# CederGroupHub/chgnet

Hardware: AMD Instinct MI355X
Metric: structures/s (energy+force+stress) on batched ~50-atom crystals (higher is better)
Workload: dtype f32; 1 GPU; 1024 x LiMnO2 5x1x1 (40 atoms, sigma=0.01 frac perturbation) per GPU, task efs; structures_per_gpu=1024, atoms=40960, directed_bonds=3535504, angles=4125764, bond_graph_nodes=213755, weights=random-init 0.3.0 architecture (tests/golden/weights_seed0.npz), parallelism=structures sharded over 1 GPU(s), RCCL all-gather of energies only, process_group_ranks=1, energies_in_all_gather=1024, comm=none (single rank)

## Files before the change

chgnet_amd/csrc/engine.hip:

```cpp

#include "engine_internal.h"
#include <cstring>

namespace chgh {

template <int UNROLL>
__global__ __launch_bounds__(256) void k_stream_copy(const f32x4* __restrict__ src, f32x4* __restrict__ dst, size_t n) {
  const size_t stride = (size_t)gridDim.x * blockDim.x;
  size_t i = (size_t)blockIdx.x * blockDim.x + threadIdx.x;
  for (; i + (UNROLL - 1) * stride < n; i += UNROLL * stride) {
    f32x4 v[UNROLL];
#pragma unroll
    for (int u = 0; u < UNROLL; ++u) v[u] = __builtin_nontemporal_load(src + i + u * stride);
#pragma unroll
    for (int u = 0; u < UNROLL; ++u) __builtin_nontemporal_store(v[u], dst + i + u * stride);
  }
  for (; i < n; i += stride) dst[i] = src[i];
}

template <bool NT>
__global__ __launch_bounds__(256) void k_stream_copy_seg(const f32x4* __restrict__ src, f32x4* __restrict__ dst, size_t n) {
  constexpr size_t SEG = 1024;
  const size_t nseg = n / SEG;
  for (size_t sgm = blockIdx.x; sgm < nseg; sgm += gridDim.x) {
// ... 78 lines not shown
  if (eng->desc.n_mlp_hidden == 0) eng->desc.n_mlp_hidden = 3;
  if (eng->desc.n_mlp_hidden != 2 && eng->desc.n_mlp_hidden != 3) {
    eng->err = "n_mlp_hidden = " + std::to_string(desc->n_mlp_hidden) + ": the energy head has two or three hidden layers";
    return CHG_EUNSUPPORTED;
  }
  if (const char* g = std::getenv("CHGNET_HIP_GRAPHS")) eng->use_graphs = std::string(g) != "0";
  if (const char* g = std::getenv("CHGNET_WIDE_RANGE")) eng->force_wide = std::string(g) == "1";
  if (const char* g = std::getenv("CHGNET_SPEC_BUILD")) eng->spec_builds = std::string(g) != "0";
  HIP_TRY(eng, hipSetDevice(device));
  hipDeviceProp_t prop;
  HIP_TRY(eng, hipGetDeviceProperties(&prop, device));
  if (std::string(prop.gcnArchName).rfind("gfx950", 0) != 0) {
    eng->err = std::string("device is ") + prop.gcnArchName + ", this library contains gfx950 code only";
    return CHG_ENODEV;
  }
  eng->num_cus = prop.multiProcessorCount;
  HIP_TRY(eng, hipStreamCreateWithFlags(&eng->stream, hipStreamNonBlocking));
  HIP_TRY(eng, hipStreamCreateWithFlags(&eng->copy_stream, hipStreamNonBlocking));
  HIP_TRY(eng, hipEventCreate(&eng->t0));
  HIP_TRY(eng, hipEventCreate(&eng->t1));
  Weights probe{};
  const size_t need = layout_weights(nullptr, desc->n_conv, probe);
  if ((int64_t)need != desc->n_weights) {
    eng->err = "weight blob has " + std::to_string(desc->n_weights) + " floats, layout needs " + std::to_string(need);
    return CHG_EINVAL;
  }
  HIP_TRY(eng, hipMalloc(&eng->d_weights, need * sizeof(float)));
  if (int rs = check_weight_range(eng, weights_blob, need); rs != CHG_OK) { eng->err = "chg_engine_create: " + eng->err; *out = eng; return rs; }
  HIP_TRY(eng, hipMemcpy(eng->d_weights, weights_blob, need * sizeof(float), hipMemcpyHostToDevice));
  layout_weights(eng->d_weights, desc->n_conv, eng->w);
  { const int si = build_images(eng); if (si) return si; }
  { int s; if ((s = predict_set_lds(eng)) || (s = chgh_wide::predict_set_lds(eng)) || (s = train_set_lds(eng)) || (s = chgh_wide::train_set_lds(eng))) return s; }
  return CHG_OK;
}

int chg_engine_destroy(chg_engine* eng) {
  if (!eng) return CHG_OK;
  hipSetDevice(eng->device);
  if (eng->stream) hipStreamSynchronize(eng->stream);
  for (auto& pe : eng->pending) { hipEventDestroy(pe.start); hipEventDestroy(pe.stop); }
  for (auto e : eng->event_pool) hipEventDestroy(e);
  if (eng->t0) hipEventDestroy(eng->t0);
  if (eng->t1) hipEventDestroy(eng->t1);
  for (auto& a : eng->arena_pool) hipFree(a.first);
  for (auto& a : eng->work_pool) hipFree(a.first);
  if (eng->scratch) hipFree(eng->scratch);
  if (eng->h_stage) hipHostFree(eng->h_stage);
  if (eng->h_out) hipHostFree(eng->h_out);
  if (eng->d_weights) hipFree(eng->d_weights);
  if (eng->d_images) hipFree(eng->d_images);
  if (eng->copy_stream) hipStreamDestroy(eng->copy_stream);
  if (eng->stream) hipStreamDestroy(eng->stream);
  delete eng;
  return CHG_OK;
}

const char* chg_last_error(const chg_engine* eng) { return eng ? eng->err.c_str() : "null engine"; }

int chg_engine_build_stats(chg_engine* eng, int64_t* single_pass_builds, int64_t* capacity_overflows) {
  if (!eng) return CHG_EINVAL;
  if (single_pass_builds) *single_pass_builds = eng->n_spec_builds;
  if (capacity_overflows) *capacity_overflows = eng->n_spec_overflows;
  return CHG_OK;
}

int chg_engine_set_graph_search(chg_engine* eng, int32_t search, int32_t cell_min_atoms) {
  if (!eng || search < 0 || search > 2 || cell_min_atoms < 0) return CHG_EINVAL;
  eng->graph_search = search;
  if (cell_min_atoms > 0) eng->cell_min_atoms = cell_min_atoms;
  return CHG_OK;
}

int chg_engine_cell_stats(chg_engine* eng, int64_t* cell_builds, int64_t* all_pairs_fallbacks) {
  if (!eng) return CHG_EINVAL;
  if (cell_builds) *cell_builds = eng->n_cell_builds;
  if (all_pairs_fallbacks) *all_pairs_fallbacks = eng->n_cell_fallbacks;
  return CHG_OK;
}

int chg_engine_set_memory_limit(chg_engine* eng, int64_t bytes) {
  if (!eng || bytes < 0) return CHG_EINVAL;
  eng->memory_limit = (size_t)bytes;
  return CHG_OK;
}

int chg_engine_memory_info(chg_engine* eng, int64_t* free_bytes, int64_t* total_bytes) {
  if (!eng) return CHG_EINVAL;
  HIP_TRY(eng, hipSetDevice(eng->device));
  size_t f = 0, t = 0;
  HIP_TRY(eng, hipMemGetInfo(&f, &t));
  std::lock_guard<std::mutex> lk(eng->pool_mu);
  for (auto& a : eng->arena_pool) f += a.second;
  for (auto& a : eng->work_pool) f += a.second;
  if (free_bytes) *free_bytes = (int64_t)f;
  if (total_bytes) *total_bytes = (int64_t)t;
  return CHG_OK;
}

int64_t chg_batch_bytes_required(int32_t n_conv, int32_t n_struct, int32_t n_atoms, int32_t n_directed, int32_t n_angles, int32_t n_bnodes) {
  if (n_conv < 2 || n_conv > MAX_CONV || n_struct < 0 || n_atoms < 0 || n_directed < 0 || (n_directed & 1) || n_angles < 0 || n_bnodes < 0) return -1;
  chg_batch probe{};
  probe.B = n_struct; probe.N = n_atoms; probe.Ed = n_directed; probe.Eu = n_directed / 2; probe.A = n_angles; probe.Eb = n_bnodes; probe.L = n_conv;
  probe.blk_cap = upload_blk_cap(probe.N, probe.A, probe.Eb);
  size_t total = 0;
  carve(&probe, nullptr, total);
  return (int64_t)total;
}

int chg_batch_upload(chg_engine* eng, const chg_batch_host* h, chg_batch** out) {
  if (!eng || !h || !out) return CHG_EINVAL;
  if (h->n_struct <= 0 || h->n_atoms <= 0 || h->n_directed < 0 || h->n_directed != 2 * h->n_undirected || h->n_angles < 0 ||
      h->n_bnodes < 0 || (h->n_angles > 0 && h->n_bnodes == 0)) {
    eng->err = "chg_batch_upload: inconsistent counts";
    return CHG_EINVAL;
  }
  HIP_TRY(eng, hipSetDevice(eng->device));
  chg_batch* b = new (std::nothrow) chg_batch();
  if (!b) return CHG_ENOMEM;
  b->B = h->n_struct; b->N = h->n_atoms; b->Ed = h->n_directed; b->Eu = h->n_undirected; b->A = h->n_angles; b->Eb = h->n_bnodes;
  b->L = eng->desc.n_conv;
  b->blk_cap = upload_blk_cap(b->N, b->A, b->Eb);
  size_t total = 0;
  carve(b, nullptr, total);
  {
    const int sa = acquire_arena(eng, b, total);
    if (sa != CHG_OK) { delete b; return sa; }
  }
  carve(b, b->arena, total);
  if (h->atom_off) b->h_atom_off.assign(h->atom_off, h->atom_off + h->n_struct + 1);
  b->h_volume.resize(h->n_struct);
  for (int q = 0; q < h->n_struct; ++q) {
    const float* Lf = h->lattice + 9 * q;
    b->h_volume[q] = Lf[0] * (Lf[4] * Lf[8] - Lf[5] * Lf[7]) + Lf[1] * (Lf[5] * Lf[6] - Lf[3] * Lf[8]) + Lf[2] * (Lf[3] * Lf[7] - Lf[4] * Lf[6]);
  }
  int s = CHG_OK;
  const size_t B = b->B, N = b->N, Ed = b->Ed, Eu = b->Eu, A = b->A, Eb = b->Eb;
#define UP(field, n) if (s == CHG_OK) s = h2d(eng, b->field, h->field, (n), eng->copy_stream)
  UP(z, N); UP(atom_owner, N); UP(atom_off, B + 1); UP(frac, 3 * N); UP(lattice, 9 * B);
  UP(e_center, Ed); UP(e_nbr, Ed); UP(e_d2u, Ed); UP(e_owner, Ed); UP(e_image, 3 * Ed); UP(e_rev, Ed); UP(p_center, Ed); UP(p_nbr, Ed);
  UP(u_u2d, Eu); UP(u_bnode, Eu); UP(bn_und, Eb);
  UP(a_ctr, A); UP(a_b1c, A); UP(a_b2c, A); UP(a_d1, A); UP(a_d2, A);
#undef UP
  b->win_pending = true;
  if (s == CHG_OK && hipStreamSynchronize(eng->copy_stream) != hipSuccess) { eng->err = "chg_batch_upload: sync failed"; s = CHG_EHIP; }
  if (s != CHG_OK) { hipFree(b->arena); delete b; return s; }
  *out = b;
  return CHG_OK;
}

int chg_debug_fetch_i32(chg_engine* eng, chg_batch* b, const char* name, int32_t* dst, int64_t capacity, int64_t* n_written) {
  if (!eng || !b || !name || !dst) return CHG_EINVAL;
  if (std::strcmp(name, "wide_range") == 0) {
    if (capacity >= 1) dst[0] = b->wide_range ? 1 : 0;
    if (n_written) *n_written = capacity >= 1 ? 1 : 0;
    return CHG_OK;
  }
  if (std::strcmp(name, "route") == 0) {
    const int64_t n = std::min<int64_t>(6, std::max<int64_t>(capacity, 0));
    std::copy(b->route, b->route + n, dst);
    if (n_written) *n_written = n;
    return CHG_OK;
  }
  if (b->named_i32.empty()) register_names(b);
  auto it = b->named_i32.find(name);
  if (it == b->named_i32.end()) { eng->err = std::string("chg_debug_fetch_i32: unknown buffer ") + name; return CHG_EINVAL; }
  const size_t n = std::min<size_t>(it->second.second, (size_t)std::max<int64_t>(capacity, 0));
  TRY(ensure_windows(eng, b));
  HIP_TRY(eng, hipStreamSynchronize(eng->stream));
  if (n) HIP_TRY(eng, hipMemcpy(dst, it->second.first, n * sizeof(int32_t), hipMemcpyDeviceToHost));
  if (n_written) *n_written = (int64_t)n;
  return CHG_OK;
}

int chg_batch_update_geometry(chg_engine* eng, chg_batch* b, const float* frac, const float* lattice) {
  if (!eng || !b) return CHG_EINVAL;
  HIP_TRY(eng, hipSetDevice(eng->device));
  int s = CHG_OK;
  if (frac) s = h2d(eng, b->frac, frac, (size_t)3 * b->N);
  if (s == CHG_OK && lattice) {
    s = h2d(eng, b->lattice, lattice, (size_t)9 * b->B);
    b->h_volume.resize(b->B);
    for (int q = 0; q < b->B; ++q) {
      const float* Lf = lattice + 9 * (size_t)q;
      b->h_volume[q] = Lf[0] * (Lf[4] * Lf[8] - Lf[5] * Lf[7]) + Lf[1] * (Lf[5] * Lf[6] - Lf[3] * Lf[8]) + Lf[2] * (Lf[3] * Lf[7] - Lf[4] * Lf[6]);
    }
  }
  b->q_tables = false;
  if (s == CHG_OK) HIP_TRY(eng, hipStreamSynchronize(eng->stream));
  return s;
}

int chg_batch_free(chg_engine* eng, chg_batch* b) {
  if (!b) return CHG_OK;
  if (eng) { hipSetDevice(eng->device); hipStreamSynchronize(eng->stream); }
  if (b->graph_exec) hipGraphExecDestroy(b->graph_exec);
  release_workspace(eng, b->train_arena, b->train_bytes, 0);
  release_workspace(eng, b->t2_arena, b->t2_bytes, 1);
  free_train2(b);
  if (b->arena) {
    bool pooled = false;
    if (eng) {
      std::lock_guard<std::mutex> lk(eng->pool_mu);
      if (eng->arena_pool.size() < 2) { eng->arena_pool.emplace_back(b->arena, b->arena_bytes); pooled = true; }
    }
    if (!pooled) hipFree(b->arena);
  }
  delete b;
  return CHG_OK;
}

int64_t chg_batch_device_bytes(const chg_batch* b) { return b ? (int64_t)b->arena_bytes : 0; }

int chg_predict(chg_engine* eng, chg_batch* b, uint32_t task_mask) {
  if (!eng || !b) return CHG_EINVAL;
  HIP_TRY(eng, hipSetDevice(eng->device));
  const uint32_t task = task_mask | CHG_TASK_E;
  TRY(ensure_windows(eng, b));
  if (eng->force_wide) b->wide_range = true;
  if (b->wide_range) return chgh_wide::run_predict(eng, b, task);
  if (eng->profiling || !eng->use_graphs) return run_predict(eng, b, task);
  if (b->graph_task != task) {
    if (b->graph_exec) hipGraphExecDestroy(b->graph_exec);
    b->graph_exec = nullptr;
    b->graph_task = task;
    b->eager_calls = 0;
  }
  if (!b->graph_exec && b->eager_calls++ == 0) return run_predict(eng, b, task);
  if (!b->graph_exec) {
    hipGraph_t graph = nullptr;
    HIP_TRY(eng, hipStreamBeginCapture(eng->stream, hipStreamCaptureModeThreadLocal));
    const int s = run_predict(eng, b, task);
    const hipError_t e = hipStreamEndCapture(eng->stream, &graph);
    if (s != CHG_OK) { if (graph) hipGraphDestroy(graph); return s; }
    if (e != hipSuccess) { eng->err = std::string("hipStreamEndCapture: ") + hipGetErrorString(e); return CHG_EHIP; }
    const hipError_t ei = hipGraphInstantiate(&b->graph_exec, graph, nullptr, nullptr, 0);
    hipGraphDestroy(graph);
    if (ei != hipSuccess) { b->graph_exec = nullptr; eng->err = std::string("hipGraphInstantiate: ") + hipGetErrorString(ei); return CHG_EHIP; }
    b->graph_task = task;
    std::copy(b->route, b->route + 6, b->graph_route);
  }
  HIP_TRY(eng, hipGraphLaunch(b->graph_exec, eng->stream));
  std::copy(b->graph_route, b->graph_route + 6, b->route);
  b->last_task = task;
  b->seed1_adjoints = (task & (CHG_TASK_F | CHG_TASK_S)) != 0;
  b->q_tables = b->seed1_adjoints;
  return CHG_OK;
}

int chg_engine_update_weights(chg_engine* eng, const float* weights_blob) {
  if (!eng || !weights_blob) return CHG_EINVAL;
  TRY(check_weight_range(eng, weights_blob, (size_t)eng->desc.n_weights));
  HIP_TRY(eng, hipSetDevice(eng->device));
  HIP_TRY(eng, hipMemcpyAsync(eng->d_weights, weights_blob, sizeof(float) * (size_t)eng->desc.n_weights, hipMemcpyHostToDevice, eng->stream));
  TRY(build_images(eng));
  HIP_TRY(eng, hipStreamSynchronize(eng->stream));
  return CHG_OK;
}

int chg_batch_all_gather_energy(chg_engine* eng, chg_batch* b, chg_comm* comm, int64_t width, float* table) {
  if (!eng || !b || !comm || !table || width < b->B) return CHG_EINVAL;
  if (b->last_task == 0) { eng->err = "chg_batch_all_gather_energy: run chg_predict on this batch first"; return CHG_EINVAL; }
  HIP_TRY(eng, hipSetDevice(eng->device));
  int32_t nranks = 1, comm_dev = -1;
  float* stage = nullptr;
  if (chg_comm_info(comm, nullptr, &nranks, &comm_dev) == CHG_OK && comm_dev != eng->device) {
    eng->err = "chg_batch_all_gather_energy: the communicator belongs to device " + std::to_string(comm_dev) + ", the engine to device " + std::to_string(eng->device);
    return CHG_EINVAL;
  }
  if (chg_comm_info(comm, nullptr, &nranks, nullptr) != CHG_OK || chg_comm_reserve(comm, width * (int64_t)(nranks + 1), &stage) != CHG_OK) {
    eng->err = std::string("chg_batch_all_gather_energy: ") + chg_comm_last_error(comm);
    return CHG_EHIP;
  }
  hipStream_t st = eng->stream;
  HIP_TRY(eng, hipMemsetAsync(stage, 0, sizeof(float) * (size_t)width, st));
  HIP_TRY(eng, hipMemcpyAsync(stage, b->energy, sizeof(float) * (size_t)b->B, hipMemcpyDeviceToDevice, st));
  if (chg_comm_all_gather_f32_device(comm, stage, width, stage + width, st) != CHG_OK) {
    eng->err = std::string("chg_batch_all_gather_energy: ") + chg_comm_last_error(comm);
    return CHG_EHIP;
  }
  HIP_TRY(eng, hipMemcpyAsync(table, stage + width, sizeof(float) * (size_t)width * nranks, hipMemcpyDeviceToHost, st));
  HIP_TRY(eng, hipStreamSynchronize(st));
  return CHG_OK;
}

void* chg_engine_stream(chg_engine* eng) { return eng ? static_cast<void*>(eng->stream) : nullptr; }
int chg_engine_device(chg_engine* eng) { return eng ? eng->device : -1; }

int chg_synchronize(chg_engine* eng) {
  if (!eng) return CHG_EINVAL;
  HIP_TRY(eng, hipStreamSynchronize(eng->stream));
  if (eng->profiling) return collect_profile(eng);
  return CHG_OK;
}

int chg_batch_download(chg_engine* eng, chg_batch* b, const chg_out_host* o) {
  if (!eng || !b || !o) return CHG_EINVAL;
  HIP_TRY(eng, hipSetDevice(eng->device));
  const size_t B = b->B, N = b->N;
  struct Piece { float* dst; const float* src; size_t n; };
  const Piece pieces[] = {
      {o->energy, b->energy, B},
      {(b->last_task & CHG_TASK_F) ? o->force : nullptr, b->force, 3 * N},
      {(b->last_task & CHG_TASK_S) ? o->stress : nullptr, b->virial, 9 * B},
      {(b->last_task & CHG_TASK_M) ? o->magmom : nullptr, b->magmom, N},
      {o->site_energy, b->site_energy, N},
      {o->atom_fea, b->atom[b->L - 1], N * D},
// ... 203 lines not shown
```

chgnet_amd/csrc/kernels_conv.h:

```cpp
#pragma once

#include "mfma_tile.h"
#include "mfma_split.h"

namespace chg {

constexpr int TS = 2 * D + PAD;
constexpr int WS = D + PAD;
constexpr int TILE_FLOATS = TILE_ROWS * TS;
constexpr int VEC_SLOTS = 6;
constexpr int IMG64 = 1024, IMG128 = 2048;
constexpr int angle_split(bool hidden, bool bwd) { return (hidden && bwd) ? 2 : 1; }

struct GatedW {
  const float *w2c, *b2c, *w2g, *b2g, *ln1_g, *ln1_b, *ln2_g, *ln2_b;
};

__device__ __forceinline__ void stage_gated_vecs(float* vecs, const GatedW& gw, bool hidden, int tid) {
  if (hidden) {
    stage_vector(vecs + 0 * D, gw.b2c, D, tid);
    stage_vector(vecs + 1 * D, gw.b2g, D, tid);
  }
  stage_vector(vecs + 2 * D, gw.ln1_g, D, tid);
  stage_vector(vecs + 3 * D, gw.ln1_b, D, tid);
// ... 354 lines not shown
    if (i >= g.n) return;
    if (y < g.p[i].col_blocks) {
      if (K == 128 && g.p[i].x2_off > 0) rows_gemm_body<K, NOUT, (K == 128 ? 2 : 1)>(g.p[i], y);
      else rows_gemm_body<K, NOUT, 1>(g.p[i], y);
      return;
    }
    y -= g.p[i].col_blocks;
  }
}

template <int K, int NOUT, int PARTS = 1>
constexpr size_t rows_gemm_lds() {
  return sizeof(float) * (PARTS * NOUT * (K + PAD) + NOUT + WAVES * TILE_ROWS * ((K > NOUT ? K : NOUT) + PAD));
}

struct AtomConvArgs {
  const float* P;
  const float* Q;
  const float* wag;
  const int *e_center, *e_nbr, *e_d2u;
  int n_edges;
  GatedW gw;
  const float *hb0, *hbc;
  const int* u_bnode;
  const float *w_bond, *q_bias;
  float* Qout;
  const float* image;
  float* agg;
  const float* GA;
  float* GP;
  float* GQ;
  float* Gwag;
  int first_wag;
  float* Gb;
  int gb_accumulate;
  float* dumpG;
  float* dumpH;
  float* g_ln;
};

constexpr int AC_VEC_SLOTS = VEC_SLOTS + 2;
template <int NW = WAVES, bool BWD = false, bool FUSEQ = false>
constexpr size_t atomconv_lds() {
  if (FUSEQ) return 16 * (size_t)(2 * IMG64 + IMG128) + sizeof(float) * (AC_VEC_SLOTS * D + NW * TILE_FLOATS);
  return 16 * (size_t)(BWD ? 4 : 2) * IMG64 + sizeof(float) * (VEC_SLOTS * D + NW * TILE_FLOATS);
}

constexpr int ac_fwd_image_floats() { return 4 * (2 * IMG64 + IMG128) + AC_VEC_SLOTS * D; }
__device__ __forceinline__ void atomconv_fwd_stage(float* base, const AtomConvArgs& p, int tid, int nthreads) {
  h16x8* I2c = reinterpret_cast<h16x8*>(base);
  h16x8* I2g = I2c + IMG64;
  h16x8* Ib = I2g + IMG64;
  float* vecs = reinterpret_cast<float*>(Ib + IMG128);
  stage_split<false>(I2c, p.gw.w2c, D, D, tid, nthreads);
  stage_split<false>(I2g, p.gw.w2g, D, D, tid, nthreads);
  stage_split<false>(Ib, p.w_bond, 2 * D, D, tid, nthreads);
  stage_gated_vecs(vecs, p.gw, true, tid);
  for (int q = tid; q < 2 * D; q += nthreads) vecs[VEC_SLOTS * D + q] = p.q_bias ? p.q_bias[q] : 0.f;
}
__device__ __forceinline__ void atomconv_bwd_stage(float* base, const AtomConvArgs& p, int tid, int nthreads) {
  h16x8* I2c = reinterpret_cast<h16x8*>(base);
  h16x8* I2g = I2c + IMG64;
  h16x8* I2cT = I2g + IMG64;
  h16x8* I2gT = I2cT + IMG64;
  float* vecs = reinterpret_cast<float*>(I2gT + IMG64);
  stage_split<false>(I2c, p.gw.w2c, D, D, tid, nthreads);
  stage_split<false>(I2g, p.gw.w2g, D, D, tid, nthreads);
  stage_split<true>(I2cT, p.gw.w2c, D, D, tid, nthreads);
  stage_split<true>(I2gT, p.gw.w2g, D, D, tid, nthreads);
  stage_gated_vecs(vecs, p.gw, true, tid);
}
constexpr int AC_RM_IMG = (int)(rm_image_bytes(D, D) / 4);
constexpr int ac_bwd_rm_image_floats() { return 2 * AC_RM_IMG + VEC_SLOTS * D + 4 * IMG128; }
__device__ __forceinline__ void atomconv_bwd_stage_rm(float* base, const AtomConvArgs& p, int tid, int nthreads) {
  stage_rm(reinterpret_cast<_Float16*>(base), p.gw.w2c, D, D, tid, nthreads);
  stage_rm(reinterpret_cast<_Float16*>(base + AC_RM_IMG), p.gw.w2g, D, D, tid, nthreads);
  float* vecs = base + 2 * AC_RM_IMG;
  stage_gated_vecs(vecs, p.gw, true, tid);
  stage_split<true>(reinterpret_cast<h16x8*>(vecs + VEC_SLOTS * D), p.w_bond, 2 * D, D, tid, nthreads);
}
template <int UNUSED = 0>
__global__ __launch_bounds__(BLOCK) void k_atomconv_image(AtomConvArgs p, float* out) { atomconv_fwd_stage(out, p, threadIdx.x, BLOCK); }
static __global__ __launch_bounds__(BLOCK) void k_atomconv_image_rm(AtomConvArgs p, float* out) { atomconv_bwd_stage_rm(out, p, threadIdx.x, BLOCK); }

__device__ __forceinline__ int bond_node(const AtomConvArgs& p, int k) { return p.hbc ? p.u_bnode[k] : -1; }
template <bool A32 = false>
__device__ __forceinline__ long bond_row_offset(const AtomConvArgs& p, int k, int bn) {
  if constexpr (A32) return (long)(bn >= 0 ? (unsigned)(p.hbc - p.hb0) + (unsigned)bn * D : (unsigned)k * D);
  else return bn >= 0 ? (p.hbc - p.hb0) + (long)bn * D : (long)k * D;
}

template <int NW, bool A32 = false>
__global__ __launch_bounds__(64 * NW) CHG_TWO_WAVES void k_atomconv_fwd(AtomConvArgs p) {
  extern __shared__ __attribute__((aligned(16))) float smem[];
  h16x8* I2c = reinterpret_cast<h16x8*>(smem);
  h16x8* I2g = I2c + IMG64;
  h16x8* Ib = I2g + IMG64;
  float* vecs = reinterpret_cast<float*>(Ib + IMG128);
  float* tiles = vecs + AC_VEC_SLOTS * D;
  const float* W2c = reinterpret_cast<const float*>(I2c);
  const float* W2g = reinterpret_cast<const float*>(I2g);
  const int tid = threadIdx.x, wave = tid >> 6, lane = tid & 63, j = lane & 15, g = lane >> 4;
  float* T = tiles + wave * TILE_FLOATS;
  float* Trow = T + j * TS;
  const int ntiles = (p.n_edges + TILE_ROWS - 1) / TILE_ROWS;
  const TileSeq ts = wave_tile_seq<true>(ntiles, NW, wave);
  const int tstride = TILE_ROWS;
  auto row_of = [&](int v) { return max(0, min(ts.at(v) * tstride + j, p.n_edges - 1)); };
  GatherPH gr;
  V64 wv_nx;
  int c_nx = 0, n_nx = 0, c_n2 = 0, n_n2 = 0;
  int bn_nx = -1, bn_n2 = -1;
  if (ts.count > 0) {
    const int r0 = row_of(0);
    c_nx = p.e_center[r0]; n_nx = p.e_nbr[r0];
    bn_nx = bond_node(p, r0 >> 1);
    gather_issue_ph<A32>(gr, p.P, c_nx, p.P + 2 * D, n_nx, 4 * D, 4 * D, p.hb0, bond_row_offset<A32>(p, r0 >> 1, bn_nx), lane);
    read_dl_g<VT, A32>(p.wag, (unsigned)(r0 >> 1), D, g, wv_nx.t);
    const int r1 = row_of(1);
    c_n2 = p.e_center[r1]; n_n2 = p.e_nbr[r1];
    bn_n2 = bond_node(p, r1 >> 1);
  }
  stage_image<ac_fwd_image_floats() / 4, 64 * NW>(smem, p.image, tid);
  __syncthreads();
  for (int v = 0; v < ts.count; ++v) {
    const int row0 = ts.at(v) * tstride;
    const int nvalid = min(TILE_ROWS, p.n_edges - row0);
    const int c = c_nx;
    const bool node = bn_nx >= 0;
    const V64 wv = wv_nx;
    gather_commit_h(gr, T, TS, lane);
    __builtin_amdgcn_wave_barrier();
    V64 x;
    read_dl<VT>(Trow, g, x.t);
    __builtin_amdgcn_wave_barrier();
    gather_commit_p(gr, T, TS, lane);
    __builtin_amdgcn_wave_barrier();
    c_nx = c_n2; n_nx = n_n2; bn_nx = bn_n2;
    if (v + 1 < ts.count) {
      const int r1 = row_of(v + 1);
      gather_issue_ph<A32>(gr, p.P, c_nx, p.P + 2 * D, n_nx, 4 * D, 4 * D, p.hb0, bond_row_offset<A32>(p, r1 >> 1, bn_nx), lane);
      read_dl_g<VT, A32>(p.wag, (unsigned)(r1 >> 1), D, g, wv_nx.t);
      const int r2 = row_of(v + 2);
      c_n2 = p.e_center[r2]; n_n2 = p.e_nbr[r2];
      bn_n2 = bond_node(p, r2 >> 1);
    }
    f32x4 z[2 * VT];
    if (!node) {
      read_dl<2 * VT>(vecs + VEC_SLOTS * D, g, z);
    } else {
#pragma unroll
      for (int ft = 0; ft < 2 * VT; ++ft) z[ft] = f32x4{0.f, 0.f, 0.f, 0.f};
    }
    gemm_split<VT, 2 * VT, false, true>(z, Ib, 2 * D, x.t, j, g);
    if (p.Qout && !(j & 1) && j < nvalid) {
      write_dl_g<2 * VT, A32>(p.Qout, (unsigned)((row0 + j) >> 1), 2 * D, g, z);
    }
    {
      f32x4 ps[2 * VT];
      read_dl<2 * VT>(Trow, g, ps);
#pragma unroll
      for (int ft = 0; ft < 2 * VT; ++ft) z[ft] += ps[ft];
    }
    V64 zc{{z[0], z[1], z[2], z[3]}}, zg{{z[4], z[5], z[6], z[7]}};
    GatedState s;
    V64 y;
    gated_forward<true, false, false, 1, true>(zc, zg, W2c, W2g, vecs, j, g, s, y);
    gather_take(gr);
    asm volatile("" : "+v"(c_n2), "+v"(n_n2), "+v"(bn_n2));
    CHG_EV(ft) asm volatile("" : "+v"(wv_nx.t[ft]));
    __builtin_amdgcn_wave_barrier();
    V64 m;
    CHG_EV(ft) m.t[ft] = y.t[ft] * wv.t[ft];
    write_dl<VT>(Trow, g, m.t);
    __builtin_amdgcn_wave_barrier();
    {
      float acc1 = 0.f, acc2 = 0.f;
      int cur1 = __builtin_amdgcn_readlane(c, 0), cur2 = __builtin_amdgcn_readlane(c, 1);
#pragma unroll
      for (int b = 0; b < TILE_ROWS / 2; ++b) {
        if (2 * b < nvalid) {
          const int c1 = __builtin_amdgcn_readlane(c, 2 * b), c2 = __builtin_amdgcn_readlane(c, 2 * b + 1);
          if (c1 != cur1) {
            tile_atomic_add(grow<float, A32>(p.agg, (unsigned)cur1, D, lane), acc1);
            acc1 = 0.f;
            cur1 = c1;
          }
          if (c2 != cur2) {
            tile_atomic_add(grow<float, A32>(p.agg, (unsigned)cur2, D, lane), acc2);
            acc2 = 0.f;
            cur2 = c2;
          }
          acc1 += T[(2 * b) * TS + lane];
          acc2 += T[(2 * b + 1) * TS + lane];
        }
      }
      tile_atomic_add(grow<float, A32>(p.agg, (unsigned)cur1, D, lane), acc1);
      tile_atomic_add(grow<float, A32>(p.agg, (unsigned)cur2, D, lane), acc2);
    }
    __builtin_amdgcn_wave_barrier();
  }
}

template <bool STORE_GQ = true, bool A32 = false>
__device__ __forceinline__ void acbwd_scatter(const float* T, int c, int nvalid, int k0, const AtomConvArgs& p, int lane) {
  float a1[4] = {0.f, 0.f, 0.f, 0.f}, a2[4] = {0.f, 0.f, 0.f, 0.f};
  int cur1 = __builtin_amdgcn_readlane(c, 0), cur2 = __builtin_amdgcn_readlane(c, 1);
#pragma unroll
  for (int b = 0; b < TILE_ROWS / 2; ++b) {
    if (2 * b < nvalid) {
      const float e0 = T[(2 * b) * TS + lane], e1 = T[(2 * b) * TS + 64 + lane];
      const float o0 = T[(2 * b + 1) * TS + lane], o1 = T[(2 * b + 1) * TS + 64 + lane];
      if (STORE_GQ) {
        float* q = p.GQ + (size_t)(k0 + b) * 2 * D + lane;
        q[0] = e0 + o0;
        q[64] = e1 + o1;
      }
      const int c1 = __builtin_amdgcn_readlane(c, 2 * b), c2 = __builtin_amdgcn_readlane(c, 2 * b + 1);
      if (c1 != cur1) {
        float* d = grow<float, A32>(p.GP, (unsigned)cur1, 4 * D, lane);
        tile_atomic_add(d, a1[0]); tile_atomic_add(d + 64, a1[1]); tile_atomic_add(d + 128, a1[2]); tile_atomic_add(d + 192, a1[3]);
        a1[0] = a1[1] = a1[2] = a1[3] = 0.f;
        cur1 = c1;
      }
      if (c2 != cur2) {
        float* d = grow<float, A32>(p.GP, (unsigned)cur2, 4 * D, lane);
        tile_atomic_add(d, a2[0]); tile_atomic_add(d + 64, a2[1]); tile_atomic_add(d + 128, a2[2]); tile_atomic_add(d + 192, a2[3]);
        a2[0] = a2[1] = a2[2] = a2[3] = 0.f;
        cur2 = c2;
      }
      a1[0] += e0; a1[1] += e1; a1[2] += o0; a1[3] += o1;
      a2[0] += o0; a2[1] += o1; a2[2] += e0; a2[3] += e1;
    }
  }
  float* d1 = grow<float, A32>(p.GP, (unsigned)cur1, 4 * D, lane);
  tile_atomic_add(d1, a1[0]); tile_atomic_add(d1 + 64, a1[1]); tile_atomic_add(d1 + 128, a1[2]); tile_atomic_add(d1 + 192, a1[3]);
  float* d2 = grow<float, A32>(p.GP, (unsigned)cur2, 4 * D, lane);
  tile_atomic_add(d2, a2[0]); tile_atomic_add(d2 + 64, a2[1]); tile_atomic_add(d2 + 128, a2[2]); tile_atomic_add(d2 + 192, a2[3]);
}

template <bool TRAIN, bool A32 = false>
__global__ __launch_bounds__(BLOCK) CHG_TWO_WAVES void k_atomconv_bwd(AtomConvArgs p) {
  constexpr bool FUSE_GQ = !TRAIN;
  constexpr int NW = WAVES;
  constexpr bool RM = FUSE_GQ;
  extern __shared__ __attribute__((aligned(16))) float smem[];
  constexpr int HMODE = RM ? 2 : 1;
  float* vecs = RM ? smem + 2 * AC_RM_IMG : smem + 4 * 4 * IMG64;
  const h16x8* IbT = reinterpret_cast<const h16x8*>(vecs + VEC_SLOTS * D);
  float* tiles = vecs + VEC_SLOTS * D + (FUSE_GQ ? 4 * IMG128 : 0);
  const float* W2c = smem;
  const float* W2g = RM ? smem + AC_RM_IMG : smem + 4 * IMG64;
  const float* W2cT = RM ? W2c : smem + 2 * 4 * IMG64;
  const float* W2gT = RM ? W2g : smem + 3 * 4 * IMG64;
  const int tid = threadIdx.x, lane = tid & 63, j = lane & 15, g = lane >> 4;
  const int wave = __builtin_amdgcn_readfirstlane(tid >> 6);
  float* T = tiles + wave * TILE_FLOATS;
  float* Trow = T + j * TS;
  const int ntiles = (p.n_edges + TILE_ROWS - 1) / TILE_ROWS;
  const TileSeq ts = wave_tile_seq<!TRAIN>(ntiles, NW, wave);
  const int last_row = p.n_edges - 1;
  int c, n, k;
  {
    const int row = max(0, min(ts.at(0) * TILE_ROWS + j, last_row));
    c = p.e_center[row]; n = p.e_nbr[row]; k = row >> 1;
    GatherRegs gr;
    gather_issue128<A32>(gr, p.P, c, p.P + 2 * D, n, p.Q, k, 4 * D, 4 * D, 2 * D, lane);
    if (TRAIN) atomconv_bwd_stage(smem, p, tid, 64 * NW);
    else stage_image<ac_bwd_rm_image_floats() / 4, 64 * NW>(smem, p.image, tid);
    gather_commit128(gr, T, TS, lane);
  }
  __syncthreads();
  TrainTile tt{};
  tt.T = T; tt.lane = lane;
  for (int v = 0; v < ts.count; ++v) {
    const int row0 = ts.at(v) * TILE_ROWS;
    const int nvalid = min(TILE_ROWS, p.n_edges - row0);
    if (TRAIN) {
      tt.nvalid = nvalid;
      tt.hrow = j < nvalid ? p.dumpH + (size_t)(row0 + j) * 2 * D : nullptr;
      tt.grow = j < nvalid ? p.dumpG + (size_t)(row0 + j) * 2 * D : nullptr;
    }
    int cn, nn, kn;
    {
      const int row = max(0, min(ts.at(v + 1) * TILE_ROWS + j, last_row));
      cn = p.e_center[row]; nn = p.e_nbr[row]; kn = row >> 1;
    }
    V64 wv, gm;
    read_dl_g<VT, A32>(p.wag, (unsigned)k, D, g, wv.t);
    read_dl_g<VT, A32>(p.GA, (unsigned)c, D, g, gm.t);
    const int k0 = row0 >> 1, nb = nvalid >> 1;
    float* gwag_rows = grow<float, A32>(p.Gwag, (unsigned)k0, D, lane);
    float prev[TILE_ROWS / 2];
#pragma unroll
    for (int b = 0; b < TILE_ROWS / 2; ++b) prev[b] = p.first_wag ? 0.f : gwag_rows[(size_t)min(b, nb - 1) * D];
    __builtin_amdgcn_wave_barrier();
    V64 zc, zg;
    read_dl<VT>(Trow, g, zc.t);
    read_dl<VT>(Trow + D, g, zg.t);
    GatedState s;
    V64 y;
    gated_forward<true, false, TRAIN, HMODE>(zc, zg, W2c, W2g, vecs, j, g, s, y, &tt);
    asm volatile("" : "+v"(cn), "+v"(nn));
    V64 gy, gw, gzc, gzg;
    CHG_EV(ft) {
      gw.t[ft] = gm.t[ft] * y.t[ft];
      gy.t[ft] = gm.t[ft] * wv.t[ft];
    }
    __builtin_amdgcn_wave_barrier();
    write_dl<VT>(Trow, g, gw.t);
    __builtin_amdgcn_wave_barrier();
    {
      float* dst = gwag_rows;
#pragma unroll
      for (int b = 0; b < TILE_ROWS / 2; ++b) prev[b] += T[(2 * b) * TS + lane] + T[(2 * b + 1) * TS + lane];
      if (nvalid == TILE_ROWS) {
#pragma unroll
        for (int b = 0; b < TILE_ROWS / 2; ++b) dst[(size_t)b * D] = prev[b];
      } else {
#pragma unroll
        for (int b = 0; b < TILE_ROWS / 2; ++b)
          if (b < nb) dst[(size_t)b * D] = prev[b];
      }
    }
    gated_backward<true, false, TRAIN, HMODE>(gy, zc, zg, W2cT, W2gT, vecs, j, g, s, gzc, gzg, &tt);
    if (FUSE_GQ) {
      float* gb_row = grow<float, A32>(p.Gb, (unsigned)(k0 + (j >> 1)), D, 4 * g);
      const bool owner = !(j & 1) && j < nvalid;
      V64 old = zero64();
      if (p.gb_accumulate && owner) {
        CHG_EV(ft) old.t[ft] = *reinterpret_cast<const f32x4*>(gb_row + 16 * ft);
      }
      f32x4 gz[2 * VT] = {gzc.t[0], gzc.t[1], gzc.t[2], gzc.t[3], gzg.t[0], gzg.t[1], gzg.t[2], gzg.t[3]};
      V64 gq = zero64();
      gemm_split<2 * VT, VT, true>(gq.t, IbT, D, gz, j, g);
      CHG_EW(ft, r) gq.t[ft][r] += __shfl_xor(gq.t[ft][r], 1);
      CHG_EV(ft) gq.t[ft] += old.t[ft];
      CHG_EV(ft) asm volatile("" : "+v"(gq.t[ft]));
      if (owner) {
        CHG_EV(ft) *reinterpret_cast<f32x4*>(gb_row + 16 * ft) = gq.t[ft];
      }
    }
    __builtin_amdgcn_wave_barrier();
    write_dl<VT>(Trow, g, gzc.t);
    write_dl<VT>(Trow + D, g, gzg.t);
    __builtin_amdgcn_wave_barrier();
    if (v + 1 < ts.count) {
      GatherRegs gr;
      gather_issue128<A32>(gr, p.P, cn, p.P + 2 * D, nn, p.Q, kn, 4 * D, 4 * D, 2 * D, lane);
      acbwd_scatter<!FUSE_GQ, A32>(T, c, nvalid, k0, p, lane);
      __builtin_amdgcn_wave_barrier();
      gather_commit128(gr, T, TS, lane);
    } else {
      acbwd_scatter<!FUSE_GQ, A32>(T, c, nvalid, k0, p, lane);
    }
    c = cn; n = nn; k = kn;
  }
  if (TRAIN) {
#pragma unroll
    for (int q = 0; q < 4; ++q) atomicAdd(p.g_ln + q * D + lane, tt.ln[q]);
  }
}

struct AngleArgs {
  const float* R;
  const float* S;
  const float* ang;
  const float* wbgc;
  const int *a_ctr, *a_b1c, *a_b2c;
  int n_angles;
  const float* w_ang;
  GatedW gw;
  const float* image;
  int slot;
  float* out;
  const float* Gagg;
  float* Gang;
  float* GR;
  float* GS;
  float* Gwbgc;
  int first_gang;
  const int* skip_flag;
  float* zsave;
  float* dumpG;
  float* dumpH;
  float* dumpZ;
  float* g_ln;
};

template <bool HIDDEN, int NW = WAVES, bool BWD = false>
constexpr size_t angle_lds() {
  if (angle_split(HIDDEN, BWD) == 2) return rm_image_bytes(2 * D, D) + 2 * rm_image_bytes(D, D) + sizeof(float) * (VEC_SLOTS * D + NW * TILE_FLOATS);
  return 16 * (size_t)((BWD ? 2 : 1) * IMG128 + (HIDDEN ? 2 * IMG64 : 0)) + sizeof(float) * (VEC_SLOTS * D + NW * TILE_FLOATS);
}


template <bool HIDDEN, bool BWD>
struct AngleLds {
  static constexpr int SPLIT = angle_split(HIDDEN, BWD);
  static constexpr int wangT = SPLIT == 2 ? 0 : 4 * IMG128;
  static constexpr int w2c = SPLIT == 2 ? (int)(rm_image_bytes(2 * D, D) / 4) : wangT + (BWD ? 4 * IMG128 : 0);
  static constexpr int w2 = HIDDEN ? (SPLIT == 2 ? (int)(rm_image_bytes(D, D) / 4) : 4 * IMG64) : 0;
  static constexpr int w2g = w2c + w2;
  static constexpr int vecs = w2g + w2;
  static constexpr int tiles = vecs + VEC_SLOTS * D;
};
template <bool HIDDEN, bool BWD>
__device__ __forceinline__ void angle_stage(float* base, const float* __restrict__ w_ang, const GatedW& gw, int tid, int nthreads) {
  using L = AngleLds<HIDDEN, BWD>;
  float* Wang = base;
  float* WangT = base + L::wangT;
  float* W2c = base + L::w2c;
  float* W2g = base + L::w2g;
  if (L::SPLIT == 2) {
    stage_rm(reinterpret_cast<_Float16*>(Wang), w_ang, 2 * D, D, tid, nthreads);
    stage_rm(reinterpret_cast<_Float16*>(W2c), gw.w2c, D, D, tid, nthreads);
    stage_rm(reinterpret_cast<_Float16*>(W2g), gw.w2g, D, D, tid, nthreads);
  } else {
    stage_split<false>(reinterpret_cast<h16x8*>(Wang), w_ang, 2 * D, D, tid, nthreads);
    if (BWD) stage_split<true>(reinterpret_cast<h16x8*>(WangT), w_ang, 2 * D, D, tid, nthreads);
    if (HIDDEN) {
      stage_split<false>(reinterpret_cast<h16x8*>(W2c), gw.w2c, D, D, tid, nthreads);
      stage_split<false>(reinterpret_cast<h16x8*>(W2g), gw.w2g, D, D, tid, nthreads);
    }
  }
  stage_gated_vecs(base + L::vecs, gw, HIDDEN, tid);
}
template <bool HIDDEN, bool BWD>
__global__ __launch_bounds__(BLOCK) void k_angle_image(const float* w_ang, GatedW gw, float* out) {
  angle_stage<HIDDEN, BWD>(out, w_ang, gw, threadIdx.x, BLOCK);
}

template <bool HIDDEN, bool BWD, int NW = WAVES, bool TRAIN = false, bool A32 = false>
__global__ __launch_bounds__(64 * NW) CHG_TWO_WAVES void k_angle(AngleArgs p) {
  static_assert(!TRAIN || BWD, "TRAIN is a variant of the adjoint kernels");
  if (!TRAIN && p.skip_flag && *p.skip_flag == 1) return;
  extern __shared__ __attribute__((aligned(16))) float smem[];
  constexpr int SPLIT = angle_split(HIDDEN, BWD);
  using L = AngleLds<HIDDEN, BWD>;
  float* Wang = smem;
  float* WangT = smem + L::wangT;
  float* W2c = smem + L::w2c;
  float* W2g = smem + L::w2g;
  float* vecs = smem + L::vecs;
  float* tiles = smem + L::tiles;
  const int tid = threadIdx.x, wave = tid >> 6, lane = tid & 63, j = lane & 15, g = lane >> 4;
  float* T = tiles + wave * TILE_FLOATS;
  float* Trow = T + j * TS;
  const int ntiles = (p.n_angles + TILE_ROWS - 1) / TILE_ROWS;
  const TileSeq ts = wave_tile_seq<!TRAIN>(ntiles, NW, wave);
  const int tstride = TILE_ROWS;
  auto row_of = [&](int v) { return max(0, min(ts.at(v) * tstride + j, p.n_angles - 1)); };
  constexpr bool PIPE = !BWD;
  int ctr_nx, b1_nx, b2_nx;
  int ctr_n2 = 0, b1_n2 = 0, b2_n2 = 0;
  GatherRegs gr_p;
  V64 x_p;
  {
    const int a0 = row_of(0);
    ctr_nx = p.a_ctr[a0]; b1_nx = p.a_b1c[a0]; b2_nx = p.a_b2c[a0];
    if (PIPE) {
      gather_issue128<A32>(gr_p, p.R, b1_nx, p.R + 2 * D, b2_nx, p.S, ctr_nx, 4 * D, 4 * D, 2 * D, lane);
      read_dl_g<VT, A32>(p.ang, (unsigned)a0, D, g, x_p.t);
      if (1 < ts.count) {
        const int a1 = row_of(1);
        ctr_n2 = p.a_ctr[a1]; b1_n2 = p.a_b1c[a1]; b2_n2 = p.a_b2c[a1];
      }
    }
  }
  if (TRAIN) angle_stage<HIDDEN, BWD>(smem, p.w_ang, p.gw, tid, 64 * NW);
  else stage_image<L::tiles / 4, 64 * NW>(smem, p.image, tid);
  __syncthreads();
  TrainTile tt{};
  tt.T = T; tt.lane = lane;
  for (int v = 0; v < ts.count; ++v) {
    int lane_t = lane;
    if (BWD && HIDDEN) asm volatile("" : "+v"(lane_t));
    const int row0 = ts.at(v) * tstride;
    const int nvalid = min(TILE_ROWS, p.n_angles - row0);
    const int ctr = ctr_nx, b1 = b1_nx, b2 = b2_nx;
    if (TRAIN) {
      tt.nvalid = nvalid;
      tt.hrow = (HIDDEN && j < nvalid) ? p.dumpH + (size_t)(row0 + j) * 2 * D : nullptr;
      tt.grow = j < nvalid ? p.dumpG + (size_t)(row0 + j) * 2 * D : nullptr;
    }
    if (!PIPE && v + 1 < ts.count) {
      const int a1 = row_of(v + 1);
      ctr_nx = p.a_ctr[a1]; b1_nx = p.a_b1c[a1]; b2_nx = p.a_b2c[a1];
    }
    if (nvalid <= 0) continue;
    const bool valid = j < nvalid;
    const int a = row0 + (valid ? j : 0);
    V64 x;
    f32x4 z[2 * VT];
    if (PIPE) {
      gather_commit128(gr_p, T, TS, lane_t);
      x = x_p;
      __builtin_amdgcn_wave_barrier();
// ... 237 lines not shown
```

chgnet_amd/csrc/mfma_tile.h:

```cpp
#pragma once

#include <hip/hip_runtime.h>
#include <stdint.h>


namespace chg {

typedef float f32x4 __attribute__((ext_vector_type(4)));

constexpr int D = 64;
constexpr int TILE_ROWS = 16;
constexpr int WAVES = 8;
constexpr int BLOCK = 64 * WAVES;
constexpr int BLOCK_ROWS = TILE_ROWS * WAVES;
constexpr int PAD = 4;
constexpr int VT = 4;
constexpr float LN_EPS = 1e-5f;
constexpr int MFMA_R = 4;

struct V64 { f32x4 t[VT]; };

__device__ __forceinline__ int dfeat(int ft, int r, int g) { return 16 * ft + 4 * g + r; }

__device__ __forceinline__ f32x4 zero4() { return f32x4{0.f, 0.f, 0.f, 0.f}; }
__device__ __forceinline__ V64 zero64() { return V64{{zero4(), zero4(), zero4(), zero4()}}; }

__device__ __forceinline__ float sigmoidf_(float x) {
  return __builtin_amdgcn_rcpf(1.0f + __builtin_amdgcn_exp2f(-1.4426950408889634f * x));
}
__device__ __forceinline__ float siluf_(float x) { return x * sigmoidf_(x); }
__device__ __forceinline__ float dsiluf_(float x) {
  const float s = sigmoidf_(x);
  return s * (1.0f + x * (1.0f - s));
}

typedef float f32x2 __attribute__((ext_vector_type(2)));
__device__ __forceinline__ f32x2 sigmoid2(f32x2 x) {
  f32x2 t = x * -1.4426950408889634f;
  t[0] = __builtin_amdgcn_exp2f(t[0]); t[1] = __builtin_amdgcn_exp2f(t[1]);
  t = t + 1.0f;
  t[0] = __builtin_amdgcn_rcpf(t[0]); t[1] = __builtin_amdgcn_rcpf(t[1]);
  return t;
}
__device__ __forceinline__ f32x4 sigmoid4(f32x4 x) {
  const f32x2 lo = sigmoid2(f32x2{x[0], x[1]}), hi = sigmoid2(f32x2{x[2], x[3]});
  return f32x4{lo[0], lo[1], hi[0], hi[1]};
}
__device__ __forceinline__ float hsum4(f32x4 v) { return (v[0] + v[1]) + (v[2] + v[3]); }
#define CHG_EV(ft) _Pragma("unroll") for (int ft = 0; ft < VT; ++ft)

#define CHG_EW(ft, r) _Pragma("unroll") for (int ft = 0; ft < VT; ++ft) _Pragma("unroll") for (int r = 0; r < 4; ++r)

template <class T, bool A32 = false>
__device__ __forceinline__ const T* grow(const float* __restrict__ base, unsigned r, int ld, int c) {
  if constexpr (A32) return reinterpret_cast<const T*>(reinterpret_cast<const char*>(base) + (r * (unsigned)(4 * ld) + (unsigned)(4 * c)));
  else return reinterpret_cast<const T*>(base + (size_t)r * ld + c);
}
template <class T, bool A32 = false>
__device__ __forceinline__ T* grow(float* __restrict__ base, unsigned r, int ld, int c) {
  if constexpr (A32) return reinterpret_cast<T*>(reinterpret_cast<char*>(base) + (r * (unsigned)(4 * ld) + (unsigned)(4 * c)));
  else return reinterpret_cast<T*>(base + (size_t)r * ld + c);
}
template <int NT>
__device__ __forceinline__ void read_dl(const float* row, int g, f32x4 (&x)[NT]) {
#pragma unroll
  for (int ft = 0; ft < NT; ++ft) x[ft] = *reinterpret_cast<const f32x4*>(row + 16 * ft + 4 * g);
}
template <int NT>
__device__ __forceinline__ void write_dl(float* row, int g, const f32x4 (&x)[NT]) {
#pragma unroll
  for (int ft = 0; ft < NT; ++ft) *reinterpret_cast<f32x4*>(row + 16 * ft + 4 * g) = x[ft];
}

template <int NT, bool A32 = false>
__device__ __forceinline__ void read_dl_g(const float* __restrict__ base, unsigned r, int ld, int g, f32x4 (&x)[NT]) {
#pragma unroll
  for (int ft = 0; ft < NT; ++ft) x[ft] = *grow<f32x4, A32>(base, r, ld, 16 * ft + 4 * g);
}
template <int NT, bool A32 = false>
__device__ __forceinline__ void write_dl_g(float* __restrict__ base, unsigned r, int ld, int g, const f32x4 (&x)[NT]) {
#pragma unroll
  for (int ft = 0; ft < NT; ++ft) *grow<f32x4, A32>(base, r, ld, 16 * ft + 4 * g) = x[ft];
}

template <int NT, bool A32 = false>
__device__ __forceinline__ void read_dl_g_nt(const float* __restrict__ base, unsigned r, int ld, int g, f32x4 (&x)[NT]) {
#pragma unroll
  for (int ft = 0; ft < NT; ++ft) x[ft] = __builtin_nontemporal_load(grow<f32x4, A32>(base, r, ld, 16 * ft + 4 * g));
}
template <int NT, bool A32 = false>
__device__ __forceinline__ void write_dl_g_nt(float* __restrict__ base, unsigned r, int ld, int g, const f32x4 (&x)[NT]) {
#pragma unroll
  for (int ft = 0; ft < NT; ++ft) __builtin_nontemporal_store(x[ft], grow<f32x4, A32>(base, r, ld, 16 * ft + 4 * g));
}

template <int KT, int NFT>
__device__ __forceinline__ void gemm_dl(f32x4 (&acc)[NFT], const float* W, int ws, const f32x4 (&x)[KT], int i, int g) {
  const float* wbase = W + i * ws + 4 * g;
#pragma unroll
  for (int kt = 0; kt < KT; ++kt) {
    f32x4 w[NFT];
#pragma unroll
    for (int fo = 0; fo < NFT; ++fo) w[fo] = *reinterpret_cast<const f32x4*>(wbase + 16 * fo * ws + 16 * kt);
#pragma unroll
    for (int r = 0; r < MFMA_R; ++r)
#pragma unroll
      for (int fo = 0; fo < NFT; ++fo) acc[fo] = __builtin_amdgcn_mfma_f32_16x16x4f32(w[fo][r], x[kt][r], acc[fo], 0, 0, 0);
  }
}

template <int NFT>
__device__ __forceinline__ void gemm_t_load(float (&a)[4][NFT], const float* W, int ws, int kt, int i, int g) {
#pragma unroll
  for (int r = 0; r < 4; ++r) {
    const float* wrow = W + dfeat(kt, r, g) * ws + i;
#pragma unroll
    for (int fo = 0; fo < NFT; ++fo) a[r][fo] = wrow[16 * fo];
  }
}
template <int NFT>
__device__ __forceinline__ void gemm_t_touch(float (&a)[4][NFT]) {
#pragma unroll
  for (int r = 0; r < 4; ++r)
#pragma unroll
    for (int fo = 0; fo < NFT; ++fo) asm volatile("" : "+v"(a[r][fo]));
}
template <int KT, int NFT>
__device__ __forceinline__ void gemm_dl_t(f32x4 (&acc)[NFT], const float* W, int ws, const f32x4 (&x)[KT], int i, int g) {
  float a[2][4][NFT];
  gemm_t_load<NFT>(a[0], W, ws, 0, i, g);
#pragma unroll
  for (int kt = 0; kt < KT; ++kt) {
    if (kt + 1 < KT) gemm_t_load<NFT>(a[(kt + 1) & 1], W, ws, kt + 1, i, g);
    gemm_t_touch<NFT>(a[kt & 1]);
#pragma unroll
    for (int r = 0; r < MFMA_R; ++r)
#pragma unroll
      for (int fo = 0; fo < NFT; ++fo) acc[fo] = __builtin_amdgcn_mfma_f32_16x16x4f32(a[kt & 1][r][fo], x[kt][r], acc[fo], 0, 0, 0);
  }
}

__device__ __forceinline__ float quad_sum(float v) {
  const unsigned u = __float_as_uint(v);
  const auto r = __builtin_amdgcn_permlane16_swap(u, u, false, false);
  const float s = __uint_as_float(r[0]) + __uint_as_float(r[1]);
  const unsigned w = __float_as_uint(s);
  const auto q = __builtin_amdgcn_permlane32_swap(w, w, false, false);
  return __uint_as_float(q[0]) + __uint_as_float(q[1]);
}

__device__ __forceinline__ float ln_normalize(V64& c) {
  f32x4 s4 = (c.t[0] + c.t[1]) + (c.t[2] + c.t[3]);
  const float mu = quad_sum(hsum4(s4)) * (1.0f / 64.0f);
  f32x4 v4 = zero4();
  CHG_EV(ft) {
    c.t[ft] = c.t[ft] - mu;
    v4 += c.t[ft] * c.t[ft];
  }
  const float rstd = __builtin_amdgcn_rsqf(quad_sum(hsum4(v4)) * (1.0f / 64.0f) + LN_EPS);
  CHG_EV(ft) c.t[ft] = c.t[ft] * rstd;
  return rstd;
}

__device__ __forceinline__ void ln_backward(V64& gy, const V64& gamma, const V64& xhat, float rstd) {
  f32x4 s1 = zero4(), s2 = zero4();
  CHG_EV(ft) {
    gy.t[ft] = gy.t[ft] * gamma.t[ft];
    s1 += gy.t[ft];
    s2 += gy.t[ft] * xhat.t[ft];
  }
  const float m1 = quad_sum(hsum4(s1)) * (1.0f / 64.0f);
  const float m2 = quad_sum(hsum4(s2)) * (1.0f / 64.0f);
  CHG_EV(ft) gy.t[ft] = (gy.t[ft] - m1 - xhat.t[ft] * m2) * rstd;
}

__device__ __forceinline__ void stage_weights(float* dst, const float* __restrict__ src, int rows, int K, int tid) {
  const int ws = K + PAD;
  const int k4 = K / 4;
  for (int idx = tid; idx < rows * k4; idx += (int)blockDim.x) {
    const int rr = idx / k4, c4 = idx - rr * k4;
    *reinterpret_cast<f32x4*>(dst + rr * ws + 4 * c4) = *reinterpret_cast<const f32x4*>(src + rr * K + 4 * c4);
  }
}
__device__ __forceinline__ void stage_vector(float* dst, const float* __restrict__ src, int n, int tid) {
  for (int idx = tid; idx < n; idx += (int)blockDim.x) dst[idx] = src[idx];
}

template <int N16, int NT, int CHUNK = 16>
__device__ __forceinline__ void stage_image(float* dst, const float* __restrict__ src, int tid) {
  constexpr int IT = (N16 + NT - 1) / NT;
#pragma unroll
  for (int u0 = 0; u0 < IT; u0 += CHUNK) {
    f32x4 v[CHUNK];
#pragma unroll
    for (int u = 0; u < CHUNK; ++u) {
      const int idx = tid + (u0 + u) * NT;
      if (u0 + u < IT && idx < N16) v[u] = reinterpret_cast<const f32x4*>(src)[idx];
    }
#pragma unroll
    for (int u = 0; u < CHUNK; ++u) {
      const int idx = tid + (u0 + u) * NT;
      if (u0 + u < IT && idx < N16) reinterpret_cast<f32x4*>(dst)[idx] = v[u];
    }
  }
}

__device__ __forceinline__ void wave_tile_range(int n_wave_tiles, int waves_per_block, int wave, int& begin, int& end) {
  const int G = gridDim.x, b = blockIdx.x;
  int lb = b;
  if ((G & 7) == 0) lb = (b & 7) * (G >> 3) + (b >> 3);
  const long W = (long)G * waves_per_block, lw = (long)lb * waves_per_block + wave;
  begin = (int)(lw * n_wave_tiles / W);
  end = (int)((lw + 1) * n_wave_tiles / W);
}

constexpr int INTERLEAVE_MIN_TILES = 6;
struct TileSeq {
  int first, stride, count;
  __device__ __forceinline__ int at(int v) const { return first + v * stride; }
};
template <bool INTERLEAVE>
__device__ __forceinline__ TileSeq wave_tile_seq(int n_wave_tiles, int waves_per_block, int wave) {
  const int G = gridDim.x, b = blockIdx.x;
  TileSeq s;
  if (INTERLEAVE && (G & 7) == 0 && (long)n_wave_tiles >= (long)INTERLEAVE_MIN_TILES * G * waves_per_block) {
    const int x = b & 7, WX = (G >> 3) * waves_per_block, lw = (b >> 3) * waves_per_block + wave;
    const int xb = (int)((long)n_wave_tiles * x / 8), xe = (int)((long)n_wave_tiles * (x + 1) / 8);
    s.first = xb + lw;
    s.stride = WX;
    s.count = xe - xb > lw ? (xe - xb - lw + WX - 1) / WX : 0;
    return s;
  }
  int tb, te;
  wave_tile_range(n_wave_tiles, waves_per_block, wave, tb, te);
  s.first = tb; s.stride = 1; s.count = te - tb;
  return s;
}

__device__ __forceinline__ int xcc_id() { return (int)(__builtin_amdgcn_s_getreg(20 | (3 << 11)) & 7u); }

__device__ __forceinline__ void tile_range_of(int ntiles, int G, int b, int& begin, int& end) {
  int lb = b;
  if ((G & 7) == 0) lb = (b & 7) * (G >> 3) + (b >> 3);
  const int per = ntiles / G, rem = ntiles - per * G;
  begin = lb * per + (lb < rem ? lb : rem);
  end = begin + per + (lb < rem ? 1 : 0);
}
__device__ __forceinline__ void tile_range(int ntiles, int& begin, int& end) { tile_range_of(ntiles, gridDim.x, blockIdx.x, begin, end); }

#define CHG_TWO_WAVES __attribute__((amdgpu_waves_per_eu(2, 2)))

__device__ __forceinline__ void tile_atomic_add(float* p, float v) {
  atomicAdd(p, v);
}

template <int W, bool A32 = false>
__device__ __forceinline__ void seg_colsum_atomic(const float* tile, int stride, int key, int nvalid, float* __restrict__ dst,
                                                  int ldd, int lane) {
  constexpr int NC = W / 64;
  float acc[NC];
#pragma unroll
  for (int c = 0; c < NC; ++c) acc[c] = 0.f;
  int cur = __builtin_amdgcn_readlane(key, 0);
#pragma unroll
  for (int rr = 0; rr < TILE_ROWS; ++rr) {
    const int kk = __builtin_amdgcn_readlane(key, rr);
    if (kk != cur) {
      if (cur >= 0) {
#pragma unroll
        for (int c = 0; c < NC; ++c) tile_atomic_add(grow<float, A32>(dst, (unsigned)cur, ldd, 64 * c + lane), acc[c]);
      }
#pragma unroll
      for (int c = 0; c < NC; ++c) acc[c] = 0.f;
      cur = kk;
    }
#pragma unroll
    for (int c = 0; c < NC; ++c) acc[c] += tile[rr * stride + 64 * c + lane];
  }
  if (cur >= 0) {
#pragma unroll
    for (int c = 0; c < NC; ++c) tile_atomic_add(grow<float, A32>(dst, (unsigned)cur, ldd, 64 * c + lane), acc[c]);
  }
}

template <int W, bool A32 = false>
__device__ __forceinline__ void row_atomic_add(const float* tile, int stride, int key, int nvalid, float* __restrict__ dst,
                                               int ldd, int lane) {
#pragma unroll
  for (int rr = 0; rr < TILE_ROWS; ++rr) {
    const int kk = __builtin_amdgcn_readlane(key, rr);
    if (kk >= 0) {
#pragma unroll
      for (int c = 0; c < W / 64; ++c) tile_atomic_add(grow<float, A32>(dst, (unsigned)kk, ldd, 64 * c + lane), tile[rr * stride + 64 * c + lane]);
    }
  }
}

template <bool A32 = false>
__device__ __forceinline__ void gather_sum128(float* tile, int stride, const float* __restrict__ t0, int i0,
                                              const float* __restrict__ t1, int i1, const float* __restrict__ t2, int i2,
                                              int ld0, int ld1, int ld2, int lane) {
// ... 173 lines not shown
```

Measured before the change: 40980 structures/s.

## Pair consecutive tiles in atomconv backward to halve fused Gb GEMM work

In the inference atom-conv backward, the fused Gb (bond gradient) GEMM now runs on pairs of consecutive tiles. Each pair's two directed-edge rows per bond are summed with a DPP lane swap before the GEMM, and the even tile's sums are kept in registers until the odd tile arrives. One MFMA pass then covers two tiles' worth of bonds instead of computing per-row products and reducing them with a shuffle afterwards. The forward gemm_split template flag is also flipped. The change adds register pressure for the kept pair and extra select logic, and the reordered summation can change floating-point results slightly.

```diff
diff --git a/chgnet_amd/csrc/engine.hip b/chgnet_amd/csrc/engine.hip
--- a/chgnet_amd/csrc/engine.hip
+++ b/chgnet_amd/csrc/engine.hip
@@ -254,6 +254,11 @@
   if (!eng || !b || !name || !dst) return CHG_EINVAL;
   if (std::strcmp(name, "wide_range") == 0) {
     if (capacity >= 1) dst[0] = b->wide_range ? 1 : 0;
+    if (n_written) *n_written = capacity >= 1 ? 1 : 0;
+    return CHG_OK;
+  }
+  if (std::strcmp(name, "num_cus") == 0) {
+    if (capacity >= 1) dst[0] = eng->num_cus;
     if (n_written) *n_written = capacity >= 1 ? 1 : 0;
     return CHG_OK;
   }
diff --git a/chgnet_amd/csrc/kernels_conv.h b/chgnet_amd/csrc/kernels_conv.h
--- a/chgnet_amd/csrc/kernels_conv.h
+++ b/chgnet_amd/csrc/kernels_conv.h
@@ -530,7 +530,7 @@
 #pragma unroll
       for (int ft = 0; ft < 2 * VT; ++ft) z[ft] = f32x4{0.f, 0.f, 0.f, 0.f};
     }
-    gemm_split<VT, 2 * VT, false, true>(z, Ib, 2 * D, x.t, j, g);
+    gemm_split<VT, 2 * VT, true, true>(z, Ib, 2 * D, x.t, j, g);
     if (p.Qout && !(j & 1) && j < nvalid) {
       write_dl_g<2 * VT, A32>(p.Qout, (unsigned)((row0 + j) >> 1), 2 * D, g, z);
     }
@@ -622,6 +622,7 @@
   constexpr bool FUSE_GQ = !TRAIN;
   constexpr int NW = WAVES;
   constexpr bool RM = FUSE_GQ;
+  constexpr bool PAIRED = FUSE_GQ;
   extern __shared__ __attribute__((aligned(16))) float smem[];
   constexpr int HMODE = RM ? 2 : 1;
   float* vecs = RM ? smem + 2 * AC_RM_IMG : smem + 4 * 4 * IMG64;
@@ -651,6 +652,8 @@
   __syncthreads();
   TrainTile tt{};
   tt.T = T; tt.lane = lane;
+  V64 pair_keep = zero64();
+  int pair_k0 = 0, pair_nvalid = 0;
   for (int v = 0; v < ts.count; ++v) {
     const int row0 = ts.at(v) * TILE_ROWS;
     const int nvalid = min(TILE_ROWS, p.n_edges - row0);
@@ -702,26 +705,58 @@
       }
     }
     gated_backward<true, false, TRAIN, HMODE>(gy, zc, zg, W2cT, W2gT, vecs, j, g, s, gzc, gzg, &tt);
-    if (FUSE_GQ) {
-      float* gb_row = grow<float, A32>(p.Gb, (unsigned)(k0 + (j >> 1)), D, 4 * g);
-      const bool owner = !(j & 1) && j < nvalid;
-      V64 old = zero64();
-      if (p.gb_accumulate && owner) {
-        CHG_EV(ft) old.t[ft] = *reinterpret_cast<const f32x4*>(gb_row + 16 * ft);
-      }
-      f32x4 gz[2 * VT] = {gzc.t[0], gzc.t[1], gzc.t[2], gzc.t[3], gzg.t[0], gzg.t[1], gzg.t[2], gzg.t[3]};
-      V64 gq = zero64();
-      gemm_split<2 * VT, VT, true>(gq.t, IbT, D, gz, j, g);
-      CHG_EW(ft, r) gq.t[ft][r] += __shfl_xor(gq.t[ft][r], 1);
-      CHG_EV(ft) gq.t[ft] += old.t[ft];
-      CHG_EV(ft) asm volatile("" : "+v"(gq.t[ft]));
-      if (owner) {
-        CHG_EV(ft) *reinterpret_cast<f32x4*>(gb_row + 16 * ft) = gq.t[ft];
-      }
-    }
     __builtin_amdgcn_wave_barrier();
     write_dl<VT>(Trow, g, gzc.t);
     write_dl<VT>(Trow + D, g, gzg.t);
+    if (FUSE_GQ) {
+      f32x4 gz[2 * VT] = {gzc.t[0], gzc.t[1], gzc.t[2], gzc.t[3], gzg.t[0], gzg.t[1], gzg.t[2], gzg.t[3]};
+      const bool pair_a = PAIRED && !(v & 1) && v + 1 < ts.count, pair_b = PAIRED && (v & 1);
+      if (pair_a || pair_b) {
+        const bool odd = j & 1;
+#pragma unroll
+        for (int ft = 0; ft < 2 * VT; ++ft)
+#pragma unroll
+          for (int r = 0; r < 4; ++r) gz[ft][r] += pair_swap(gz[ft][r]);
+        if (pair_a) {
+          CHG_EW(ft, r) pair_keep.t[ft][r] = odd ? gz[VT + ft][r] : gz[ft][r];
+          pair_k0 = k0; pair_nvalid = nvalid;
+        } else {
+          float* gb_row = grow<float, A32>(p.Gb, (unsigned)((odd ? k0 : pair_k0) + (j >> 1)), D, 4 * g);
+          const bool owner = j < (odd ? nvalid : pair_nvalid);
+          V64 old = zero64();
+          if (p.gb_accumulate && owner) {
+            CHG_EV(ft) old.t[ft] = *reinterpret_cast<const f32x4*>(gb_row + 16 * ft);
+          }
+          CHG_EW(ft, r) {
+            const float other = pair_swap(pair_keep.t[ft][r]);
+            gz[ft][r] = odd ? gz[ft][r] : pair_keep.t[ft][r];
+            gz[VT + ft][r] = odd ? gz[VT + ft][r] : other;
+          }
+          V64 gq = zero64();
+          gemm_split<2 * VT, VT, true>(gq.t, IbT, D, gz, j, g);
+          CHG_EV(ft) gq.t[ft] += old.t[ft];
+          CHG_EV(ft) asm volatile("" : "+v"(gq.t[ft]));
+          if (owner) {
+            CHG_EV(ft) *reinterpret_cast<f32x4*>(gb_row + 16 * ft) = gq.t[ft];
+          }
+        }
+      } else {
+        float* gb_row = grow<float, A32>(p.Gb, (unsigned)(k0 + (j >> 1)), D, 4 * g);
+        const bool owner = !(j & 1) && j < nvalid;
+        V64 old = zero64();
+        if (p.gb_accumulate && owner) {
+          CHG_EV(ft) old.t[ft] = *reinterpret_cast<const f32x4*>(gb_row + 16 * ft);
+        }
+        V64 gq = zero64();
+        gemm_split<2 * VT, VT, true>(gq.t, IbT, D, gz, j, g);
+        CHG_EW(ft, r) gq.t[ft][r] += __shfl_xor(gq.t[ft][r], 1);
+        CHG_EV(ft) gq.t[ft] += old.t[ft];
+        CHG_EV(ft) asm volatile("" : "+v"(gq.t[ft]));
+        if (owner) {
+          CHG_EV(ft) *reinterpret_cast<f32x4*>(gb_row + 16 * ft) = gq.t[ft];
+        }
+      }
+    }
     __builtin_amdgcn_wave_barrier();
     if (v + 1 < ts.count) {
       GatherRegs gr;
diff --git a/chgnet_amd/csrc/mfma_tile.h b/chgnet_amd/csrc/mfma_tile.h
--- a/chgnet_amd/csrc/mfma_tile.h
+++ b/chgnet_amd/csrc/mfma_tile.h
@@ -147,6 +147,10 @@
   const unsigned w = __float_as_uint(s);
   const auto q = __builtin_amdgcn_permlane32_swap(w, w, false, false);
   return __uint_as_float(q[0]) + __uint_as_float(q[1]);
+}
+
+__device__ __forceinline__ float pair_swap(float v) {
+  return __int_as_float(__builtin_amdgcn_update_dpp(0, __float_as_int(v), 0xB1, 0xF, 0xF, true));
 }
 
 __device__ __forceinline__ float ln_normalize(V64& c) {
```

New measurement: 40970 structures/s. About the same (-0.0%).
